# UoB-HPC/stdpar-nbody

Hardware: AMD Instinct MI355X
Metric: body-steps/sec + %FP64 peak, 3D double all-pairs N=2^20 at 1/2/4/8 GPUs (higher is better)
Workload: dtype f64

## Files before the change

stdpar-nbody_amd/csrc/all_pairs.hip:

```cpp
#include "common.hpp"
#include "k1_order_key.hpp"
#include "radix_sort.hpp"

#include <atomic>
#include <cstdlib>
#include <mutex>
#include <type_traits>
#include <vector>

namespace nbody {

constexpr int kBlock = 256;
constexpr int kWaves = kBlock / 64;

struct ap_config {
  int split = 0;
  int tpt   = 0;
  int path  = 0;
};
static std::atomic<uint32_t> g_ap_default{0};

static ap_config ap_config_of(const nbody_state* s) {
  const uint32_t t = s->tuning ? s->tuning : g_ap_default.load(std::memory_order_relaxed);
  ap_config c;
// ... 24 lines not shown

template <typename T, int D>
__global__ __launch_bounds__(kBlock) void pack_sources_kernel(const T* __restrict__ m, const T* __restrict__ x,
                                                              src_rec<T, D>* __restrict__ out, uint32_t sz, uint32_t padded) {
  const uint32_t j = blockIdx.x * kBlock + threadIdx.x;
  if (j >= padded) return;
  src_rec<T, D> r;
#pragma unroll
  for (int k = 0; k < 3; ++k) r.p[k] = (k < D && j < sz) ? x[uint64_t(j) * D + (k < D ? k : 0)] : T(0);
  r.m    = j < sz ? m[j] : T(0);
  out[j] = r;
}

template <typename T>
struct k1_prepare_tail {
  uint32_t turn_words;
};
template <>
struct k1_prepare_tail<double> {
  uint32_t turn_words;
  uint32_t bpc;
  double* cbox;
  double* pbox;
};
template <typename T, int D, bool PACK, bool MOMENTS>
__global__ __launch_bounds__(kBlock) void k1_prepare_kernel(const T* __restrict__ m, const T* __restrict__ x, src_rec<T, D>* __restrict__ out,
                                                            cst_batch* __restrict__ cst, uint32_t sz, uint32_t padded, k1_rule* rule, double* partial,
                                                            uint32_t* turn, k1_prepare_tail<T> tail) {
  constexpr bool BOX        = PACK && MOMENTS && sizeof(T) == 8;
  const uint32_t turn_words = tail.turn_words;
  [[maybe_unused]] uint32_t bpc = 0;
  [[maybe_unused]] T *cbox = nullptr, *pbox = nullptr;
  if constexpr (BOX) bpc = tail.bpc, cbox = tail.cbox, pbox = tail.pbox;
  const uint32_t j = blockIdx.x * kBlock + threadIdx.x;
  T p[D];
#pragma unroll
  for (int k = 0; k < D; ++k) p[k] = j < sz ? x[uint64_t(j) * D + k] : T(0);
  if constexpr (PACK) {
    if (j < padded) {
      src_rec<T, D> r;
#pragma unroll
      for (int k = 0; k < 3; ++k) r.p[k] = k < D ? p[k < D ? k : 0] : T(0);
      r.m    = j < sz ? m[j] : T(0);
      out[j] = r;
      if constexpr (sizeof(T) == 8) {
        const src_cst<T> k  = src_cst<T>::of(r.m);
        cst[j / 2].m15[j % 2]   = k.m15;
        cst[j / 2].m1875[j % 2] = k.m1875;
      }
    }
  }
  __shared__ double red[2 * D][kWaves];
  __shared__ T bred[BOX ? 2 * D : 1][kWaves];
  __shared__ bool last_s;
  const int lane = threadIdx.x & 63, wave = threadIdx.x >> 6;
  if constexpr (MOMENTS) {
// ... 84 lines not shown
    __syncthreads();
    if (threadIdx.x < 2 * D) {
      double tot = 0.0;
#pragma unroll 6
      for (int gg = 0; gg < G; ++gg) tot += fin[gg * (2 * D) + threadIdx.x];
      fin[threadIdx.x] = tot;
    }
    __syncthreads();
    if (threadIdx.x == 0) {
      double vol = 1.0;
#pragma unroll
      for (int k = 0; k < D; ++k) {
        const double mean = fin[k] / double(sz), var = fin[D + k] / double(sz) - mean * mean;
        vol *= var > 0.0 ? __builtin_sqrt(12.0 * var) : 0.0;
      }
      rule->volume = vol;
      rule->sparse = vol >= kFarMinVolume<D> ? 1u : 0u;
    }
  }
  if constexpr (BOX) {
    if (bpc != 0) {
      const uint32_t nchunks = (gridDim.x + bpc - 1) / bpc;
      const uint32_t sub     = threadIdx.x & 15u;
      for (uint32_t c0 = 0; c0 < nchunks; c0 += kBlock / 16) {
        const uint32_t c  = c0 + (threadIdx.x >> 4);
        const uint32_t b1 = c < nchunks ? min(gridDim.x, (c + 1u) * bpc) : 0u;
        T lo[D], hi[D];
#pragma unroll
        for (int k = 0; k < D; ++k) lo[k] = T(__builtin_inf()), hi[k] = -T(__builtin_inf());
        for (uint32_t b0 = c * bpc + sub; b0 < b1; b0 += 16u * 4u) {
          T v[4][2 * D];
#pragma unroll
          for (int u = 0; u < 4; ++u) {
            const uint32_t b = b0 + 16u * uint32_t(u);
#pragma unroll
            for (int q = 0; q < 2 * D; ++q)
              v[u][q] = b < b1 ? __hip_atomic_load(pbox + size_t(b) * (2 * D) + q, __ATOMIC_RELAXED, __HIP_MEMORY_SCOPE_AGENT)
                               : (q < D ? T(__builtin_inf()) : -T(__builtin_inf()));
          }
#pragma unroll
          for (int u = 0; u < 4; ++u)
#pragma unroll
            for (int k = 0; k < D; ++k) {
              lo[k] = __builtin_fmin(lo[k], v[u][k]);
              hi[k] = __builtin_fmax(hi[k], v[u][D + k]);
            }
        }
#pragma unroll
        for (int k = 0; k < D; ++k)
          for (int off = 8; off > 0; off >>= 1) {
            lo[k] = __builtin_fmin(lo[k], __shfl_xor(lo[k], off, 64));
            hi[k] = __builtin_fmax(hi[k], __shfl_xor(hi[k], off, 64));
          }
        if (c < nchunks && sub == 0) {
#pragma unroll
          for (int k = 0; k < D; ++k) {
            cbox[size_t(c) * (2 * D) + k]     = lo[k];
            cbox[size_t(c) * (2 * D) + D + k] = hi[k];
          }
        }
      }
    }
  }
  for (uint32_t w = threadIdx.x; w < turn_words; w += kBlock) turn[w] = 0u;
  if (threadIdx.x == 0) __hip_atomic_store(&rule->ticket, 0u, __ATOMIC_RELAXED, __HIP_MEMORY_SCOPE_AGENT);
}

template <int JS>
constexpr int kSgprWaves = JS > kWaves ? JS : kWaves;

constexpr uint32_t kTurnSpins  = 1u << 26;
constexpr uint32_t kTurnPoison = 0xffffffffu;
struct k1_status {
  uint32_t err, block, group, chunk;
  unsigned long long polls, waits;
};
struct k1_handoff {
  void* sums;
  uint32_t* turn;
  k1_status* status;
  uint32_t spins;
  uint32_t delay;
  uint32_t late;
};
constexpr size_t kBoxHeaderBytes = 64;
template <typename T>
struct k1_rule_arg {
  const k1_rule* rule;
};
template <>
struct k1_rule_arg<double> {
  const k1_rule* rule;
  const double* box;
};
template <typename T, int D, int R, int JS, int RULE = 0>
__global__ __launch_bounds__(64 * kSgprWaves<JS>) void all_pairs_force_sgpr_kernel(const src_rec<T, D>* __restrict__ packed,
                                                                                   const cst_batch* __restrict__ cst,
                                                                                   const T* __restrict__ x, T* a, T c, uint32_t sz,
                                                                                   uint32_t first, uint32_t count,
                                                                                   uint32_t tiles_per_chunk, k1_handoff h,
                                                                                   k1_rule_arg<T> ra) {
  [[maybe_unused]] constexpr T e2 = T(0);
  const k1_rule* __restrict__ const rule = ra.rule;
  [[maybe_unused]] const T* __restrict__ box = nullptr;
  if constexpr (sizeof(T) == 8) box = ra.box;
#define K1_SOFT false
#include "k1_sgpr_body.inc"
#undef K1_SOFT
}
template <typename T, int D, int R, int JS>
__global__ __launch_bounds__(64 * kSgprWaves<JS>) void all_pairs_softened_sgpr_kernel(const src_rec<T, D>* __restrict__ packed,
                                                                                      const cst_batch* __restrict__ cst,
                                                                                      const T* __restrict__ x, T* a, T c, uint32_t sz,
                                                                                      uint32_t first, uint32_t count,
                                                                                      uint32_t tiles_per_chunk, k1_handoff h, T e2) {
  constexpr int RULE = 0;
  const k1_rule* const rule = nullptr;
  [[maybe_unused]] const T* const box = nullptr;
#define K1_SOFT true
#include "k1_sgpr_body.inc"
#undef K1_SOFT
}

namespace {
struct scratch_buf {
  void* ptr  = nullptr;
  size_t cap = 0;
};
struct packed_slot {
  int device;
  hipStream_t stream;
  scratch_buf buf[9];
  std::vector<void*> retired;
  bool k1_dirty  = false;
  bool k1_failed = false;
};
std::mutex g_packed_mu;
std::vector<packed_slot> g_packed_slots;
}

int ap_scratch_get(hipStream_t st, int which, size_t bytes, void** out) {
// ... 101 lines not shown
  void* scratch         = nullptr;
  if (int r = ap_scratch_get(st, 0, 4 * tsz * size_t(padded), &scratch)) return r;
  int rc = dispatch(s->dtype, s->dim, [&](auto tg) {
    using T         = typename decltype(tg)::type;
    constexpr int D = decltype(tg)::dim;
    hipLaunchKernelGGL((pack_sources_kernel<T, D>), dim3((padded + kBlock - 1) / kBlock), dim3(kBlock), 0, st,
                       static_cast<const T*>(s->m), static_cast<const T*>(s->x), static_cast<src_rec<T, D>*>(scratch), s->sz, padded);
    NB_HIP(hipGetLastError());
    return int(NBODY_OK);
  });
  *packed_out = scratch;
  return rc;
}

static size_t ap_cst_bytes(size_t padded) { return sizeof(cst_batch) * (padded / 2); }

static size_t ap_rule_bytes(uint32_t sz, int dim) {
  const size_t padded = (size_t(sz) + kTileJ - 1) / kTileJ * kTileJ;
  return 32 + sizeof(double) * 2 * size_t(dim) * (padded / kBlock);
}

static size_t ap_box_bytes(uint32_t sz, int dim) {
  const size_t ntiles = (size_t(sz) + kTileJ - 1) / kTileJ;
  return kBoxHeaderBytes + sizeof(double) * 2 * size_t(dim) * (ntiles + ntiles * (kTileJ / kBlock));
}
static bool k1_box_wanted(uint32_t sz, uint32_t chunks) { return sz >= kFarMinBodies && chunks > 1; }

constexpr double kOrderSafe = 1e150;
__device__ __forceinline__ double k1_order_safe(double p, bool on) { return on && p > kOrderSafe ? kOrderSafe : (on && p < -kOrderSafe ? -kOrderSafe : p); }
constexpr uint32_t kOrderMinBodies = 262144;
static bool k1_order_wanted(uint32_t sz, uint32_t chunks) {
  if (const char* e = experiment_env("NBODY_K1_NO_ORDER"); e && e[0] == '1') return false;
  uint32_t least = kOrderMinBodies;
  if (const char* e = experiment_env("NBODY_K1_ORDER_MIN")) least = uint32_t(strtoul(e, nullptr, 10));
  return k1_box_wanted(sz, chunks) && sz >= least;
}

struct k1_order_layout {
  size_t recs, cst, keys[2], idx[2], hist, xs, as, bytes;
};
static k1_order_layout k1_order_layout_of(uint32_t sz, uint32_t count, int dim) {
  const size_t padded = (size_t(sz) + kTileJ - 1) / kTileJ * kTileJ;
  size_t at           = 0;
  auto take = [&](size_t bytes) {
    const size_t here = at;
    at += (bytes + 255) / 256 * 256;
    return here;
// ... 54 lines not shown
    for (int off = 32; off > 0; off >>= 1) {
      lo[k] = __builtin_fmin(lo[k], __shfl_xor(lo[k], off, 64));
      hi[k] = __builtin_fmax(hi[k], __shfl_xor(hi[k], off, 64));
    }
  __shared__ double bred[2 * D][kWaves];
  const int lane = threadIdx.x & 63, wave = threadIdx.x >> 6;
  if (lane == 0) {
#pragma unroll
    for (int k = 0; k < D; ++k) {
      bred[k][wave]     = lo[k];
      bred[D + k][wave] = hi[k];
    }
  }
  __syncthreads();
  if (threadIdx.x < 2 * D) {
    const int q = int(threadIdx.x);
    double v    = bred[q][0];
    for (int w = 1; w < kWaves; ++w) v = q < D ? __builtin_fmin(v, bred[q][w]) : __builtin_fmax(v, bred[q][w]);
    pbox[size_t(blockIdx.x) * (2 * D) + q] = v;
  }
}

template <int D>
__global__ __launch_bounds__(kBlock) void k1_order_box_kernel(const double* __restrict__ pbox, uint32_t nblk, uint32_t bpc, double* __restrict__ cbox) {
  const uint32_t b0 = blockIdx.x * bpc, b1 = min(nblk, b0 + bpc);
  double lo[D], hi[D];
#pragma unroll
  for (int k = 0; k < D; ++k) lo[k] = __builtin_inf(), hi[k] = -__builtin_inf();
  for (uint32_t b = b0 + threadIdx.x; b < b1; b += kBlock) {
#pragma unroll
    for (int k = 0; k < D; ++k) {
      lo[k] = __builtin_fmin(lo[k], pbox[size_t(b) * (2 * D) + k]);
      hi[k] = __builtin_fmax(hi[k], pbox[size_t(b) * (2 * D) + D + k]);
    }
  }
#pragma unroll
  for (int k = 0; k < D; ++k)
    for (int off = 32; off > 0; off >>= 1) {
      lo[k] = __builtin_fmin(lo[k], __shfl_xor(lo[k], off, 64));
      hi[k] = __builtin_fmax(hi[k], __shfl_xor(hi[k], off, 64));
    }
  __shared__ double bred[2 * D][kWaves];
  const int lane = threadIdx.x & 63, wave = threadIdx.x >> 6;
  if (lane == 0) {
#pragma unroll
    for (int k = 0; k < D; ++k) {
      bred[k][wave]     = lo[k];
      bred[D + k][wave] = hi[k];
    }
  }
  __syncthreads();
  if (threadIdx.x < 2 * D) {
    const int q = int(threadIdx.x);
    double v    = bred[q][0];
    for (int w = 1; w < kWaves; ++w) v = q < D ? __builtin_fmin(v, bred[q][w]) : __builtin_fmax(v, bred[q][w]);
    cbox[size_t(blockIdx.x) * (2 * D) + q] = v;
  }
}

template <int D>
__global__ __launch_bounds__(kBlock) void k1_order_targets_kernel(const double* __restrict__ x, uint32_t first, uint32_t count,
                                                                  const uint32_t* __restrict__ perm, double* __restrict__ xs,
                                                                  const k1_rule* __restrict__ rule) {
  const uint32_t k = blockIdx.x * kBlock + threadIdx.x;
  if (k >= count) return;
  const uint64_t i = uint64_t(first) + perm[k];
  const bool safe  = rule->sparse != 0u;
#pragma unroll
  for (int d = 0; d < D; ++d) xs[uint64_t(k) * D + d] = k1_order_safe(x[i * D + d], safe);
}

template <int D>
__global__ __launch_bounds__(kBlock) void k1_order_scatter_kernel(const uint64_t* __restrict__ as, uint32_t count, const uint32_t* __restrict__ perm,
                                                                  uint64_t* __restrict__ a) {
  const uint32_t k = blockIdx.x * kBlock + threadIdx.x;
  if (k >= count) return;
  const uint64_t i = perm[k];
#pragma unroll
  for (int d = 0; d < D; ++d) a[i * D + d] = as[uint64_t(k) * D + d];
}

template <int D>
struct k1_ordered {
  src_rec<double, D>* packed;
  const cst_batch* cst;
  const double* box;
  const double* xs;
  double* as;
  const uint32_t* tperm;
};

template <int D>
static int k1_order_queue(const nbody_state* s, hipStream_t st, const src_rec<double, D>* packed, const cst_batch* cst, const k1_rule* rule,
                          uint32_t tpc, k1_ordered<D>* out) {
  const uint32_t padded = (s->sz + kTileJ - 1) / kTileJ * kTileJ, nblk = padded / kBlock, bpc = tpc * (kTileJ / kBlock);
  const k1_order_layout l = k1_order_layout_of(s->sz, s->count, D);
  void *w = nullptr, *b = nullptr;
  if (int r = ap_scratch_get(st, 8, l.bytes, &w)) return r;
  if (int r = ap_scratch_get(st, 7, ap_box_bytes(s->sz, D), &b)) return r;
  char* base = static_cast<char*>(w);
  uint64_t* keys[2] = {reinterpret_cast<uint64_t*>(base + l.keys[0]), reinterpret_cast<uint64_t*>(base + l.keys[1])};
  uint32_t* idx[2]  = {reinterpret_cast<uint32_t*>(base + l.idx[0]), reinterpret_cast<uint32_t*>(base + l.idx[1])};
  uint32_t* hist    = reinterpret_cast<uint32_t*>(base + l.hist);
  auto* recs        = reinterpret_cast<src_rec<double, D>*>(base + l.recs);
  auto* csts        = reinterpret_cast<cst_batch*>(base + l.cst);
  double* xs        = reinterpret_cast<double*>(base + l.xs);
  double* cbox      = reinterpret_cast<double*>(static_cast<char*>(b) + kBoxHeaderBytes);
  double* pbox      = cbox + size_t(2 * D) * (padded / kTileJ);
  const double* x   = static_cast<const double*>(s->x);
  const bool whole  = s->first == 0 && s->count == s->sz;
  int fin           = 0;
  hipLaunchKernelGGL((k1_order_key_kernel<D>), dim3((s->sz + kBlock - 1) / kBlock), dim3(kBlock), 0, st, x, 0u, s->sz, rule, keys[0]);
  NB_HIP(hipGetLastError());
  if (int r = radix_sort_pairs(keys, idx, s->sz, kOrderKeyBits, hist, st, &fin)) return r;
  hipLaunchKernelGGL((k1_order_gather_kernel<D>), dim3(nblk), dim3(kBlock), 0, st, packed, cst, idx[fin], recs, csts, s->sz, pbox,
                     whole ? xs : static_cast<double*>(nullptr), rule);
  NB_HIP(hipGetLastError());
  hipLaunchKernelGGL((k1_order_box_kernel<D>), dim3((nblk + bpc - 1) / bpc), dim3(kBlock), 0, st, pbox, nblk, bpc, cbox);
  NB_HIP(hipGetLastError());
  if (!whole) {
    hipLaunchKernelGGL((k1_order_key_kernel<D>), dim3((s->count + kBlock - 1) / kBlock), dim3(kBlock), 0, st, x, s->first, s->count, rule, keys[0]);
    NB_HIP(hipGetLastError());
    if (int r = radix_sort_pairs(keys, idx, s->count, kOrderKeyBits, hist, st, &fin)) return r;
    hipLaunchKernelGGL((k1_order_targets_kernel<D>), dim3((s->count + kBlock - 1) / kBlock), dim3(kBlock), 0, st, x, s->first, s->count, idx[fin], xs, rule);
    NB_HIP(hipGetLastError());
  }
  *out = {recs, csts, cbox, xs, reinterpret_cast<double*>(base + l.as), idx[fin]};
  return NBODY_OK;
}

template <typename T, int D>
static int ap_prepare(const nbody_state* s, hipStream_t st, bool pack, src_rec<T, D>** packed_out, const cst_batch** cst_out,
                      const k1_rule** rule_out, uint32_t* turn, size_t turn_words, bool with_rule = true, uint32_t box_tpc = 0,
                      const T** box_out = nullptr) {
  const uint32_t padded = (s->sz + kTileJ - 1) / kTileJ * kTileJ;
  const bool moments    = with_rule && s->sz >= kFarMinBodies;
  void* scratch         = nullptr;
  void* consts          = nullptr;
  if (pack) {
    if (int r = ap_scratch_get(st, 0, 4 * sizeof(T) * size_t(padded), &scratch)) return r;
    if (sizeof(T) == 8)
      if (int r = ap_scratch_get(st, 6, ap_cst_bytes(padded), &consts)) return r;
  }
  void* q = nullptr;
  if (int r = ap_scratch_get(st, 3, ap_rule_bytes(s->sz, D), &q)) return r;
  auto* rule    = static_cast<k1_rule*>(q);
  auto* partial = reinterpret_cast<double*>(static_cast<char*>(q) + 32);
  auto* out     = static_cast<src_rec<T, D>*>(scratch);
  auto* cst     = static_cast<cst_batch*>(consts);
  T *cbox = nullptr, *pbox = nullptr;
  uint32_t bpc = 0;
  if (sizeof(T) == 8 && pack && moments && box_tpc != 0) {
    void* b = nullptr;
    if (int r = ap_scratch_get(st, 7, ap_box_bytes(s->sz, D), &b)) return r;
    cbox = reinterpret_cast<T*>(static_cast<char*>(b) + kBoxHeaderBytes);
    pbox = cbox + size_t(2 * D) * (padded / kTileJ);
    bpc  = box_tpc * (kTileJ / kBlock);
  }
  const dim3 grid(padded / kBlock), block(kBlock);
  const T *m = static_cast<const T*>(s->m), *x = static_cast<const T*>(s->x);
  const uint32_t words = uint32_t(turn_words);
  k1_prepare_tail<T> tail{};
  tail.turn_words = words;
  if constexpr (sizeof(T) == 8) tail.bpc = bpc, tail.cbox = cbox, tail.pbox = pbox;
  if (pack && moments) hipLaunchKernelGGL((k1_prepare_kernel<T, D, true, true>), grid, block, 0, st, m, x, out, cst, s->sz, padded, rule, partial, turn, tail);
  else if (pack) hipLaunchKernelGGL((k1_prepare_kernel<T, D, true, false>), grid, block, 0, st, m, x, out, cst, s->sz, padded, rule, partial, turn, tail);
  else if (moments) hipLaunchKernelGGL((k1_prepare_kernel<T, D, false, true>), grid, block, 0, st, m, x, out, cst, s->sz, padded, rule, partial, turn, tail);
  NB_HIP(hipGetLastError());
  if (box_out) *box_out = cbox;
  if (packed_out) *packed_out = out;
  if (cst_out) *cst_out = cst;
  *rule_out = moments ? rule : nullptr;
  return NBODY_OK;
}

constexpr uint32_t kCollectMaxBlocks = 2048;
static bool k1_collect(uint32_t target_blocks, uint32_t chunks) {
  uint32_t limit = kCollectMaxBlocks;
  if (const char* e = experiment_env("NBODY_K1_COLLECT_MAX")) limit = uint32_t(atoi(e));
  return chunks > 1 && uint64_t(target_blocks) * chunks <= limit;
}
template <typename T, int D, int R, int JS>
static size_t k1_collect_bytes(uint32_t target_blocks, uint32_t chunks) {
  constexpr int TG = kSgprWaves<JS> / JS;
  return sizeof(T) * size_t(chunks) * target_blocks * TG * R * D * 64;
}

template <int R, int JS>
static size_t sgpr_turn_words(uint32_t count) {
  constexpr int TG = kSgprWaves<JS> / JS, TB = TG * 64 * R;
  return size_t((count + TB - 1) / TB) * TG;
}
// ... 7 lines not shown
  if (plan.chunks > 1) {
    void* q = nullptr;
    if (int r = ap_scratch_get(st, 1, sizeof(uint32_t) * sgpr_turn_words<R, JS>(s->count), &q)) return r;
    h.turn = static_cast<uint32_t*>(q);
    if (k1_collect(blocks, plan.chunks)) {
      if (int r = ap_scratch_get(st, 5, k1_collect_bytes<T, D, R, JS>(blocks, plan.chunks), &q)) return r;
      h.sums = q;
    }
    if (int r = ap_scratch_get(st, 4, sizeof(k1_status), &q)) return r;
    h.status = static_cast<k1_status*>(q);
    if (const char* e = experiment_env("NBODY_K1_TURN_SPINS")) h.spins = uint32_t(strtoul(e, nullptr, 10));
    if (const char* e = experiment_env("NBODY_K1_HANDOFF_DELAY")) h.delay = uint32_t(strtoul(e, nullptr, 10));
    if (const char* e = experiment_env("NBODY_K1_HANDOFF_LATE")) h.late = uint32_t(strtoul(e, nullptr, 10));
    if (const char* e = experiment_env("NBODY_K1_NO_HANDOFF"); e && e[0] == '1') h.turn = nullptr, h.sums = nullptr;
    if (const char* e = experiment_env("NBODY_K1_COLLECT"); e && e[0] == '0') h.sums = nullptr;
  }
  src_rec<T, D>* packed = nullptr;
  const cst_batch* cst  = nullptr;
  const k1_rule* rule   = nullptr;
  const T* box          = nullptr;
  bool certify          = !SOFT && sizeof(T) == 8 && k1_box_wanted(s->sz, plan.chunks);
  if (const char* e = experiment_env("NBODY_K1_NO_CERT"); e && e[0] == '1') certify = false;
  [[maybe_unused]] const bool ordered = certify && plan.chunks > 1 && k1_order_wanted(s->sz, plan.chunks);
  if (int r = ap_prepare<T, D>(s, st, true, &packed, &cst, &rule, h.turn, h.turn ? sgpr_turn_words<R, JS>(s->count) : 0, !SOFT,
                               certify && !ordered ? plan.tiles_per_chunk : 0u, &box))
    return r;
  if constexpr (SOFT) {
    hipLaunchKernelGGL((all_pairs_softened_sgpr_kernel<T, D, R, JS>), dim3(blocks, plan.chunks), dim3(64 * kSgprWaves<JS>), 0, st,
                       packed, cst, static_cast<const T*>(s->x), static_cast<T*>(s->a), static_cast<T>(s->c), s->sz, s->first, s->count,
                       plan.tiles_per_chunk, h, e2);
    NB_HIP(hipGetLastError());
    if (h.turn != nullptr && h.sums == nullptr) ap_status_mark(st);
    return NBODY_OK;
  }
  k1_rule_arg<T> ra{};
  ra.rule = rule;
  if constexpr (sizeof(T) == 8) ra.box = box;
#ifdef NBODY_EXPERIMENTS
  if (const char* e = getenv("NBODY_K1_RULE_FORCE"); e && JS == 8 && D == 3) {
    if (e[0] == '1')
      hipLaunchKernelGGL((all_pairs_force_sgpr_kernel<T, D, R, JS, 1>), dim3(blocks, plan.chunks), dim3(64 * kSgprWaves<JS>), 0, st,
                         packed, cst, static_cast<const T*>(s->x), static_cast<T*>(s->a), static_cast<T>(s->c), s->sz, s->first, s->count,
                         plan.tiles_per_chunk, h, ra);
    else
      hipLaunchKernelGGL((all_pairs_force_sgpr_kernel<T, D, R, JS, 2>), dim3(blocks, plan.chunks), dim3(64 * kSgprWaves<JS>), 0, st,
                         packed, cst, static_cast<const T*>(s->x), static_cast<T*>(s->a), static_cast<T>(s->c), s->sz, s->first, s->count,
                         plan.tiles_per_chunk, h, ra);
    NB_HIP(hipGetLastError());
    return NBODY_OK;
  }
#endif
  if constexpr (sizeof(T) == 8) {
    if (ordered) {
      k1_ordered<D> o{};
      if (int r = k1_order_queue<D>(s, st, packed, cst, rule, plan.tiles_per_chunk, &o)) return r;
      ra.box = o.box;
      hipLaunchKernelGGL((all_pairs_force_sgpr_kernel<T, D, R, JS>), dim3(blocks, plan.chunks), dim3(64 * kSgprWaves<JS>), 0, st,
                         o.packed, o.cst, o.xs, o.as, static_cast<T>(s->c), s->sz, 0u, s->count, plan.tiles_per_chunk, h, ra);
      NB_HIP(hipGetLastError());
      hipLaunchKernelGGL((k1_order_scatter_kernel<D>), dim3((s->count + kBlock - 1) / kBlock), dim3(kBlock), 0, st,
                         reinterpret_cast<const uint64_t*>(o.as), s->count, o.tperm, static_cast<uint64_t*>(s->a));
      NB_HIP(hipGetLastError());
      if (h.turn != nullptr && h.sums == nullptr) ap_status_mark(st);
      return NBODY_OK;
    }
  }
  hipLaunchKernelGGL((all_pairs_force_sgpr_kernel<T, D, R, JS>), dim3(blocks, plan.chunks), dim3(64 * kSgprWaves<JS>), 0, st,
                     packed, cst, static_cast<const T*>(s->x), static_cast<T*>(s->a), static_cast<T>(s->c), s->sz, s->first, s->count,
                     plan.tiles_per_chunk, h, ra);
  NB_HIP(hipGetLastError());
  if (h.turn != nullptr && h.sums == nullptr) ap_status_mark(st);
  return NBODY_OK;
}

template <typename T, int D, int R, int JS, bool SOFT>
static int launch_all_pairs(const nbody_state* s, hipStream_t st, T e2) {
  constexpr int TB = (kWaves / JS) * 64 * R;
  uint32_t blocks  = (s->count + TB - 1) / TB;
  if (blocks == 0) return NBODY_OK;
// ... 42 lines not shown
    rc = p.scalar ? launch_all_pairs_sgpr<T, D, R, JS, SOFT>(s, p, st, e2)
                  : (JS <= kWaves ? launch_all_pairs<T, D, R, (JS <= kWaves ? JS : 1), SOFT>(s, st, e2) : int(NBODY_ERR_ARG));
  });
  if (!found) {
    set_error("all-pairs: unsupported config split=%d targets_per_thread=%d", p.js, p.r);
    return NBODY_ERR_ARG;
  }
  return rc;
}

template <typename T, int D>
static int all_pairs_describe(const nbody_state* s, char* out, size_t len) {
  k1_plan p;
  if (int rc = plan_all_pairs<T>(s, &p)) return rc;
  const char* t = sizeof(T) == 8 ? "double" : "float";
  const char* pair = sizeof(T) == 4 ? (s->sz >= kFarMinBodies ? "rsq+rcp[m y^3 at r2 >= 4 if sparse]" : "rsq+rcp")
                                    : s->sz >= kFarMinBodies ? "far3m[-eps if sparse]/near3" : "far3m/near3";
  if (p.scalar) {
    bool collect = false;
    with_k1_instance(p, [&](auto r, auto js) {
      constexpr int TB = (kSgprWaves<decltype(js)::value> / decltype(js)::value) * 64 * decltype(r)::value;
      collect = k1_collect((s->count + TB - 1) / TB, p.chunks);
    });
    snprintf(out, len, "all_pairs_force_sgpr_kernel<%s,%d,R=%d,JS=%d> tile=%d chunks=%u%s pair=%s%s", t, D, p.r, p.js, kTileJ, p.chunks,
             p.chunks > 1 ? (collect ? "(summed in chunk order by the last to arrive)" : "(summed in turn into a)") : "", pair,
             sizeof(T) == 8 && k1_box_wanted(s->sz, p.chunks)
                 ? (k1_order_wanted(s->sz, p.chunks) ? " cert=box-gap>=3[if sparse: blocks proven far skip the r2 test] order=morton30[if sparse]"
                                                    : " cert=box-gap>=3[if sparse: blocks proven far skip the r2 test]")
                 : "");
  }
  else
    snprintf(out, len, "all_pairs_force_kernel<%s,%d,R=%d,JS=%d> tile=%d chunks=1 pair=%s", t, D, p.r, p.js, kTileJ, pair);
  return NBODY_OK;
}

int ap_scratch_reserve(hipStream_t st, const nbody_state* s) {
  void* q             = nullptr;
  const size_t tsz    = s->dtype == NBODY_F32 ? 4 : 8;
  const size_t padded = (size_t(s->sz) + 2 * kTileJ - 1) / (2 * kTileJ) * (2 * kTileJ);
  if (int r = ap_scratch_get(st, 0, 4 * tsz * padded, &q)) return r;
  if (s->dtype == NBODY_F64)
    if (int r = ap_scratch_get(st, 6, ap_cst_bytes(padded), &q)) return r;
  if (int r = ap_scratch_get(st, 3, ap_rule_bytes(s->sz, s->dim), &q)) return r;
  if (s->dtype == NBODY_F64 && s->sz >= kFarMinBodies)
    if (int r = ap_scratch_get(st, 7, ap_box_bytes(s->sz, s->dim), &q)) return r;
  if (s->dtype == NBODY_F64) {
    k1_plan p;
    if (int rc = plan_all_pairs<double>(s, &p)) return rc;
    if (p.scalar && k1_order_wanted(s->sz, p.chunks))
      if (int r = ap_scratch_get(st, 8, k1_order_layout_of(s->sz, s->count, s->dim).bytes, &q)) return r;
  }
  return dispatch(s->dtype, s->dim, [&](auto tg) {
// ... 653 lines not shown

extern "C" int nbody_all_pairs_softened_force(const nbody_state* s, double eps, void* stream) {
  if (int r = check_state(s)) return r;
  return dispatch(s->dtype, s->dim, [&](auto tg) {
    using TG = decltype(tg);
    using T  = typename TG::type;
    T e2;
    if (int r = check_softening<T>(eps, &e2)) return r;
    device_guard guard(stream_device(as_stream(stream)));
    return all_pairs_dispatch<T, TG::dim, true>(s, as_stream(stream), e2);
  });
}

extern "C" int nbody_all_pairs_status(void* stream, uint64_t out[6], int clear) {
  device_guard guard(stream_device(as_stream(stream)));
  unsigned long long v[6] = {0, 0, 0, 0, 0, 0};
  const int rc = ap_status_read(as_stream(stream), v, clear != 0);
  if (out)
    for (int i = 0; i < 6; ++i) out[i] = v[i];
  return rc;
}

#ifdef NBODY_EXPERIMENTS
extern "C" int nbody_exp_k1_certified(void* stream, uint64_t* out, int clear) {
  NB_ARG(out != nullptr, "out is NULL");
  hipStream_t st = as_stream(stream);
  const int dev  = stream_device(st);
  device_guard guard(dev);
  void* dptr = nullptr;
  {
    std::lock_guard<std::mutex> lock(g_packed_mu);
    for (auto& sl : g_packed_slots)
      if (sl.stream == st && sl.device == dev) dptr = sl.buf[7].ptr;
  }
  unsigned long long v = 0;
  if (dptr) NB_HIP(hipMemcpyAsync(&v, dptr, sizeof v, hipMemcpyDeviceToHost, st));
  NB_HIP(hipStreamSynchronize(st));
  if (dptr && clear) {
    NB_HIP(hipMemsetAsync(dptr, 0, sizeof v, st));
    NB_HIP(hipStreamSynchronize(st));
  }
  *out = v;
  return NBODY_OK;
}
#endif

extern "C" int nbody_all_pairs_collapsed_force(const nbody_state* s, void* stream) {
  if (int r = check_state(s)) return r;
  device_guard guard(stream_device(as_stream(stream)));
  return dispatch(s->dtype, s->dim, [&](auto tg) {
    using TG = decltype(tg);
    return collapsed_dispatch<typename TG::type, TG::dim>(s, as_stream(stream));
  });
}

extern "C" int nbody_accelerate_step(const nbody_state* s, void* stream) {
  if (int r = check_state(s)) return r;
// ... 7 lines not shown
```

stdpar-nbody_amd/csrc/k1_sgpr_body.inc:

```
  using rec_t = src_rec<T, D>;
  constexpr int TG  = kSgprWaves<JS> / JS;
  constexpr int TB  = TG * 64 * R;
  constexpr int SUB = kTileJ / JS;
  __shared__ T partial[(JS > 1) ? (JS - 1) * TG * 64 * R * D : 1];
  const int lane   = threadIdx.x & 63;
  const int wave   = __builtin_amdgcn_readfirstlane(threadIdx.x >> 6);
  const int tgroup = wave / JS;
  const int jpart  = wave % JS;
  T xi[R][D], acc[R][D];
  uint32_t ti[R];
#pragma unroll
  for (int r = 0; r < R; ++r) {
    uint32_t local = blockIdx.x * TB + tgroup * (64 * R) + r * 64 + lane;
    ti[r]          = local;
    uint64_t i     = uint64_t(first) + (local < count ? local : 0u);
#pragma unroll
    for (int k = 0; k < D; ++k) {
      xi[r][k]  = x[i * D + k];
      acc[r][k] = T(0);
    }
  }
  const uint32_t ntiles = (sz + kTileJ - 1) / kTileJ;
  const uint32_t t0     = blockIdx.y * tiles_per_chunk;
  const uint32_t t1     = min(ntiles, t0 + tiles_per_chunk);
  const pair_consts<T> pc;
  const bool ffar       = !K1_SOFT && ap_far_mode(rule);
  const uint32_t nsteps = (t1 - t0) * SUB;
  constexpr int U = 64 / int(sizeof(rec_t));
  struct batch_t {
    rec_t r[U];
  };
  auto batch = [&](uint32_t k) { return packed + (uint64_t(t0 + k / SUB) * kTileJ + uint32_t(jpart) * SUB + (k % SUB)); };
  constexpr bool CST = sizeof(T) == 8;
  auto cbatch = [&](uint32_t k) { return cst + (uint64_t(t0 + k / SUB) * kTileJ + uint32_t(jpart) * SUB + (k % SUB)) / U; };
  [[maybe_unused]] uint32_t vzero = 0;
  if constexpr (CST) {
    asm volatile("" : "+v"(vzero));
#pragma unroll
    for (int r = 0; r < R; ++r)
#pragma unroll
      for (int k = 0; k < D; ++k) asm volatile("" : "+v"(xi[r][k]));
  }
  [[maybe_unused]] bool cfar = false;
  if constexpr (!K1_SOFT && CST && RULE == 0) {
    if (ffar && box != nullptr) {
      cfar = k1_block_is_far<T, D, R>(xi, (const T __attribute__((address_space(4)))*)(box + size_t(blockIdx.y) * (2 * D)));
#ifdef NBODY_EXPERIMENTS
      if (cfar && jpart == 0 && lane == 0)
        atomicAdd(reinterpret_cast<unsigned long long*>(const_cast<T*>(box)) - kBoxHeaderBytes / 8, 1ull);
#endif
    }
  }
  auto run = [&](auto ff) {
    constexpr int FF = int(decltype(ff)::value);
    sgpr16 A, B;
    [[maybe_unused]] cst_regs CA, CB;
    auto request = [&](sgpr16& S, cst_regs& C, uint32_t k) {
      if constexpr (CST) C = cload(cbatch(k), vzero, xi[0][0]);
      S = sload16(batch(k), xi[0][0]);
    };
    auto wait = [&](sgpr16& S, cst_regs& C) {
      if constexpr (CST) cswait(S, C, acc[0][0]);
      else swait(S, acc[0][0]);
    };
    auto consume = [&](const sgpr16& S, const cst_regs& C) {
      const batch_t b = __builtin_bit_cast(batch_t, S);
      src_cst<T> kc[U];
      if constexpr (CST) cst_unpack(C, kc);
      if constexpr (K1_SOFT) pair_batch_soft<T, D, R, U, true>(acc, xi, b.r, kc, pc, e2);
      else if constexpr (FF == 2) pair_batch_far<T, D, R, U>(acc, xi, b.r, kc);
      else pair_batch<T, D, R, U, FF != 0>(acc, xi, b.r, kc, pc);
    };
    request(A, CA, 0);
    for (uint32_t k = 0; k < nsteps; k += 2 * U) {
      wait(A, CA);
      request(B, CB, k + U);
      consume(A, CA);
      wait(B, CB);
      request(A, CA, k + 2 * U < nsteps ? k + 2 * U : k);
      consume(B, CB);
    }
    wait(A, CA);
  };
  if constexpr (K1_SOFT) run(std::false_type{});
  else if constexpr (RULE == 1) run(std::false_type{});
  else if constexpr (RULE == 2) run(std::true_type{});
  else if (ffar) {
    if constexpr (CST) {
      if (cfar) run(std::integral_constant<int, 2>{});
      else run(std::true_type{});
    } else run(std::true_type{});
  } else run(std::false_type{});
  if constexpr (JS > 1) {
    if (jpart > 0) {
#pragma unroll
      for (int r = 0; r < R; ++r)
#pragma unroll
        for (int k = 0; k < D; ++k) partial[((((jpart - 1) * TG + tgroup) * R + r) * D + k) * 64 + lane] = acc[r][k];
    }
    __syncthreads();
    if (jpart == 0) {
#pragma unroll
      for (int p = 1; p < JS; ++p)
#pragma unroll
        for (int r = 0; r < R; ++r)
#pragma unroll
          for (int k = 0; k < D; ++k) acc[r][k] += partial[((((p - 1) * TG + tgroup) * R + r) * D + k) * 64 + lane];
    }
  }
  if (jpart != 0) return;
  const uint32_t y = blockIdx.y, last = gridDim.y - 1u;
  uint32_t* const tw = h.turn + blockIdx.x * TG + tgroup;
  if (h.sums != nullptr) {
    const size_t group_scalars = size_t(R) * D * 64;
    T* const all  = static_cast<T*>(h.sums);
// ... 112 lines not shown
```

Before: 1.829 million.

## Certify far-field at finer tile-run granularity to skip distance tests per run

Adds per-run bounding boxes (groups of tiles within a chunk) computed in the prepare and order-box kernels. When a whole chunk is not proven far, the force kernel now tests each run separately and uses the cheaper far-field pair routine for runs proven far, splitting the main loop into segments. This aims to skip more r2 tests in sparse configurations, at the cost of extra box reduction work, more box checks per block, and a segmented loop with a restarted prefetch pipeline at each run boundary.

```diff
diff --git a/stdpar-nbody_amd/csrc/all_pairs.hip b/stdpar-nbody_amd/csrc/all_pairs.hip
--- a/stdpar-nbody_amd/csrc/all_pairs.hip
+++ b/stdpar-nbody_amd/csrc/all_pairs.hip
@@ -70,6 +70,9 @@
   uint32_t bpc;
   double* cbox;
   double* pbox;
+  uint32_t bpr;
+  uint32_t rpc;
+  double* rbox;
 };
 template <typename T, int D, bool PACK, bool MOMENTS>
 __global__ __launch_bounds__(kBlock) void k1_prepare_kernel(const T* __restrict__ m, const T* __restrict__ x, src_rec<T, D>* __restrict__ out,
@@ -78,8 +81,9 @@
   constexpr bool BOX        = PACK && MOMENTS && sizeof(T) == 8;
   const uint32_t turn_words = tail.turn_words;
   [[maybe_unused]] uint32_t bpc = 0;
-  [[maybe_unused]] T *cbox = nullptr, *pbox = nullptr;
-  if constexpr (BOX) bpc = tail.bpc, cbox = tail.cbox, pbox = tail.pbox;
+  [[maybe_unused]] T *cbox = nullptr, *pbox = nullptr, *rbox = nullptr;
+  [[maybe_unused]] uint32_t bpr = 0, rpc = 1;
+  if constexpr (BOX) bpc = tail.bpc, cbox = tail.cbox, pbox = tail.pbox, bpr = tail.bpr, rpc = tail.rpc, rbox = tail.rbox;
   const uint32_t j = blockIdx.x * kBlock + threadIdx.x;
   T p[D];
 #pragma unroll
@@ -210,44 +214,50 @@
     if (bpc != 0) {
       const uint32_t nchunks = (gridDim.x + bpc - 1) / bpc;
       const uint32_t sub     = threadIdx.x & 15u;
-      for (uint32_t c0 = 0; c0 < nchunks; c0 += kBlock / 16) {
-        const uint32_t c  = c0 + (threadIdx.x >> 4);
-        const uint32_t b1 = c < nchunks ? min(gridDim.x, (c + 1u) * bpc) : 0u;
-        T lo[D], hi[D];
-#pragma unroll
-        for (int k = 0; k < D; ++k) lo[k] = T(__builtin_inf()), hi[k] = -T(__builtin_inf());
-        for (uint32_t b0 = c * bpc + sub; b0 < b1; b0 += 16u * 4u) {
-          T v[4][2 * D];
-#pragma unroll
-          for (int u = 0; u < 4; ++u) {
-            const uint32_t b = b0 + 16u * uint32_t(u);
-#pragma unroll
-            for (int q = 0; q < 2 * D; ++q)
-              v[u][q] = b < b1 ? __hip_atomic_load(pbox + size_t(b) * (2 * D) + q, __ATOMIC_RELAXED, __HIP_MEMORY_SCOPE_AGENT)
-                               : (q < D ? T(__builtin_inf()) : -T(__builtin_inf()));
+      auto reduce = [&](uint32_t per, uint32_t width, T* dst) {
+        const uint32_t units = nchunks * per;
+        for (uint32_t c0 = 0; c0 < units; c0 += kBlock / 16) {
+          const uint32_t c  = c0 + (threadIdx.x >> 4);
+          const uint32_t at = (c / per) * bpc + (c % per) * width;
+          const uint32_t b1 = c < units ? min(gridDim.x, min(at + width, (c / per + 1u) * bpc)) : 0u;
+          T lo[D], hi[D];
+#pragma unroll
+          for (int k = 0; k < D; ++k) lo[k] = T(__builtin_inf()), hi[k] = -T(__builtin_inf());
+          for (uint32_t b0 = at + sub; b0 < b1; b0 += 16u * 4u) {
+            T v[4][2 * D];
+#pragma unroll
+            for (int u = 0; u < 4; ++u) {
+              const uint32_t b = b0 + 16u * uint32_t(u);
+#pragma unroll
+              for (int q = 0; q < 2 * D; ++q)
+                v[u][q] = b < b1 ? __hip_atomic_load(pbox + size_t(b) * (2 * D) + q, __ATOMIC_RELAXED, __HIP_MEMORY_SCOPE_AGENT)
+                                 : (q < D ? T(__builtin_inf()) : -T(__builtin_inf()));
+            }
+#pragma unroll
+            for (int u = 0; u < 4; ++u)
+#pragma unroll
+              for (int k = 0; k < D; ++k) {
+                lo[k] = __builtin_fmin(lo[k], v[u][k]);
+                hi[k] = __builtin_fmax(hi[k], v[u][D + k]);
+              }
           }
 #pragma unroll
-          for (int u = 0; u < 4; ++u)
+          for (int k = 0; k < D; ++k)
+            for (int off = 8; off > 0; off >>= 1) {
+              lo[k] = __builtin_fmin(lo[k], __shfl_xor(lo[k], off, 64));
+              hi[k] = __builtin_fmax(hi[k], __shfl_xor(hi[k], off, 64));
+            }
+          if (c < units && sub == 0) {
 #pragma unroll
             for (int k = 0; k < D; ++k) {
-              lo[k] = __builtin_fmin(lo[k], v[u][k]);
-              hi[k] = __builtin_fmax(hi[k], v[u][D + k]);
+              dst[size_t(c) * (2 * D) + k]     = lo[k];
+              dst[size_t(c) * (2 * D) + D + k] = hi[k];
             }
-        }
-#pragma unroll
-        for (int k = 0; k < D; ++k)
-          for (int off = 8; off > 0; off >>= 1) {
-            lo[k] = __builtin_fmin(lo[k], __shfl_xor(lo[k], off, 64));
-            hi[k] = __builtin_fmax(hi[k], __shfl_xor(hi[k], off, 64));
-          }
-        if (c < nchunks && sub == 0) {
-#pragma unroll
-          for (int k = 0; k < D; ++k) {
-            cbox[size_t(c) * (2 * D) + k]     = lo[k];
-            cbox[size_t(c) * (2 * D) + D + k] = hi[k];
           }
         }
-      }
+      };
+      reduce(1u, bpc, cbox);
+      if (bpr != 0) reduce(rpc, bpr, rbox);
     }
   }
   for (uint32_t w = threadIdx.x; w < turn_words; w += kBlock) turn[w] = 0u;
@@ -280,7 +290,25 @@
 struct k1_rule_arg<double> {
   const k1_rule* rule;
   const double* box;
+  const double* rbox;
+  uint32_t cert_tiles;
+  uint32_t runs_per_chunk;
 };
+constexpr uint32_t kCertTiles = 16;
+struct k1_runs {
+  uint32_t tiles = 0, per_chunk = 1;
+};
+static k1_runs k1_runs_of(uint32_t tiles_per_chunk) {
+  uint32_t ct = kCertTiles;
+  if (const char* e = experiment_env("NBODY_K1_CERT_TILES")) ct = uint32_t(atoi(e));
+  const uint32_t least = (tiles_per_chunk + 63) / 64;
+  if (ct < least) ct = least;
+  k1_runs r;
+  if (ct == 0 || ct >= tiles_per_chunk) return r;
+  r.tiles     = ct;
+  r.per_chunk = (tiles_per_chunk + ct - 1) / ct;
+  return r;
+}
 template <typename T, int D, int R, int JS, int RULE = 0>
 __global__ __launch_bounds__(64 * kSgprWaves<JS>) void all_pairs_force_sgpr_kernel(const src_rec<T, D>* __restrict__ packed,
                                                                                    const cst_batch* __restrict__ cst,
@@ -291,7 +319,9 @@
   [[maybe_unused]] constexpr T e2 = T(0);
   const k1_rule* __restrict__ const rule = ra.rule;
   [[maybe_unused]] const T* __restrict__ box = nullptr;
-  if constexpr (sizeof(T) == 8) box = ra.box;
+  [[maybe_unused]] const T* __restrict__ rbox = nullptr;
+  [[maybe_unused]] uint32_t cert_tiles = 0, runs_per_chunk = 1;
+  if constexpr (sizeof(T) == 8) box = ra.box, rbox = ra.rbox, cert_tiles = ra.cert_tiles, runs_per_chunk = ra.runs_per_chunk;
 #define K1_SOFT false
 #include "k1_sgpr_body.inc"
 #undef K1_SOFT
@@ -304,7 +334,8 @@
                                                                                       uint32_t tiles_per_chunk, k1_handoff h, T e2) {
   constexpr int RULE = 0;
   const k1_rule* const rule = nullptr;
-  [[maybe_unused]] const T* const box = nullptr;
+  [[maybe_unused]] const T *const box = nullptr, *const rbox = nullptr;
+  [[maybe_unused]] constexpr uint32_t cert_tiles = 1, runs_per_chunk = 1;
 #define K1_SOFT true
 #include "k1_sgpr_body.inc"
 #undef K1_SOFT
@@ -452,7 +483,14 @@
 
 static size_t ap_box_bytes(uint32_t sz, int dim) {
   const size_t ntiles = (size_t(sz) + kTileJ - 1) / kTileJ;
-  return kBoxHeaderBytes + sizeof(double) * 2 * size_t(dim) * (ntiles + ntiles * (kTileJ / kBlock));
+  return kBoxHeaderBytes + sizeof(double) * 2 * size_t(dim) * (ntiles + ntiles * (kTileJ / kBlock) + 2 * ntiles + 2);
+}
+template <int D>
+static void ap_box_arrays(void* buf, uint32_t sz, double** cbox, double** pbox, double** rbox) {
+  const size_t ntiles = (size_t(sz) + kTileJ - 1) / kTileJ;
+  *cbox = reinterpret_cast<double*>(static_cast<char*>(buf) + kBoxHeaderBytes);
+  *pbox = *cbox + size_t(2 * D) * ntiles;
+  *rbox = *pbox + size_t(2 * D) * ntiles * (kTileJ / kBlock);
 }
 static bool k1_box_wanted(uint32_t sz, uint32_t chunks) { return sz >= kFarMinBodies && chunks > 1; }
 
@@ -553,8 +591,13 @@
 }
 
 template <int D>
-__global__ __launch_bounds__(kBlock) void k1_order_box_kernel(const double* __restrict__ pbox, uint32_t nblk, uint32_t bpc, double* __restrict__ cbox) {
-  const uint32_t b0 = blockIdx.x * bpc, b1 = min(nblk, b0 + bpc);
+__global__ __launch_bounds__(kBlock) void k1_order_box_kernel(const double* __restrict__ pbox, uint32_t nblk, uint32_t bpc, double* __restrict__ cbox,
+                                                              uint32_t nchunks, uint32_t bpr, uint32_t rpc, double* __restrict__ rbox) {
+  const bool is_run = blockIdx.x >= nchunks;
+  const uint32_t u  = is_run ? blockIdx.x - nchunks : blockIdx.x;
+  const uint32_t c  = is_run ? u / rpc : u;
+  const uint32_t b0 = c * bpc + (is_run ? (u % rpc) * bpr : 0u), b1 = min(nblk, min(b0 + (is_run ? bpr : bpc), (c + 1u) * bpc));
+  double* const dst = is_run ? rbox : cbox;
   double lo[D], hi[D];
 #pragma unroll
   for (int k = 0; k < D; ++k) lo[k] = __builtin_inf(), hi[k] = -__builtin_inf();
@@ -585,7 +628,7 @@
     const int q = int(threadIdx.x);
     double v    = bred[q][0];
     for (int w = 1; w < kWaves; ++w) v = q < D ? __builtin_fmin(v, bred[q][w]) : __builtin_fmax(v, bred[q][w]);
-    cbox[size_t(blockIdx.x) * (2 * D) + q] = v;
+    dst[size_t(u) * (2 * D) + q] = v;
   }
 }
 
@@ -616,6 +659,7 @@
   src_rec<double, D>* packed;
   const cst_batch* cst;
   const double* box;
+  const double* rbox;
   const double* xs;
   double* as;
   const uint32_t* tperm;
@@ -623,7 +667,7 @@
 
 template <int D>
 static int k1_order_queue(const nbody_state* s, hipStream_t st, const src_rec<double, D>* packed, const cst_batch* cst, const k1_rule* rule,
-                          uint32_t tpc, k1_ordered<D>* out) {
+                          uint32_t tpc, const k1_runs& runs, k1_ordered<D>* out) {
   const uint32_t padded = (s->sz + kTileJ - 1) / kTileJ * kTileJ, nblk = padded / kBlock, bpc = tpc * (kTileJ / kBlock);
   const k1_order_layout l = k1_order_layout_of(s->sz, s->count, D);
   void *w = nullptr, *b = nullptr;
@@ -636,8 +680,9 @@
   auto* recs        = reinterpret_cast<src_rec<double, D>*>(base + l.recs);
   auto* csts        = reinterpret_cast<cst_batch*>(base + l.cst);
   double* xs        = reinterpret_cast<double*>(base + l.xs);
-  double* cbox      = reinterpret_cast<double*>(static_cast<char*>(b) + kBoxHeaderBytes);
-  double* pbox      = cbox + size_t(2 * D) * (padded / kTileJ);
+  double *cbox = nullptr, *pbox = nullptr, *rbox = nullptr;
+  ap_box_arrays<D>(b, s->sz, &cbox, &pbox, &rbox);
+  const uint32_t nchunks = (nblk + bpc - 1) / bpc, bpr = runs.tiles * (kTileJ / kBlock);
   const double* x   = static_cast<const double*>(s->x);
   const bool whole  = s->first == 0 && s->count == s->sz;
   int fin           = 0;
@@ -647,7 +692,8 @@
   hipLaunchKernelGGL((k1_order_gather_kernel<D>), dim3(nblk), dim3(kBlock), 0, st, packed, cst, idx[fin], recs, csts, s->sz, pbox,
                      whole ? xs : static_cast<double*>(nullptr), rule);
   NB_HIP(hipGetLastError());
-  hipLaunchKernelGGL((k1_order_box_kernel<D>), dim3((nblk + bpc - 1) / bpc), dim3(kBlock), 0, st, pbox, nblk, bpc, cbox);
+  hipLaunchKernelGGL((k1_order_box_kernel<D>), dim3(nchunks + (bpr ? nchunks * runs.per_chunk : 0u)), dim3(kBlock), 0, st, pbox, nblk, bpc, cbox,
+                     nchunks, bpr, runs.per_chunk, rbox);
   NB_HIP(hipGetLastError());
   if (!whole) {
     hipLaunchKernelGGL((k1_order_key_kernel<D>), dim3((s->count + kBlock - 1) / kBlock), dim3(kBlock), 0, st, x, s->first, s->count, rule, keys[0]);
@@ -656,14 +702,14 @@
     hipLaunchKernelGGL((k1_order_targets_kernel<D>), dim3((s->count + kBlock - 1) / kBlock), dim3(kBlock), 0, st, x, s->first, s->count, idx[fin], xs, rule);
     NB_HIP(hipGetLastError());
   }
-  *out = {recs, csts, cbox, xs, reinterpret_cast<double*>(base + l.as), idx[fin]};
+  *out = {recs, csts, cbox, bpr ? rbox : nullptr, xs, reinterpret_cast<double*>(base + l.as), idx[fin]};
   return NBODY_OK;
 }
 
 template <typename T, int D>
 static int ap_prepare(const nbody_state* s, hipStream_t st, bool pack, src_rec<T, D>** packed_out, const cst_batch** cst_out,
                       const k1_rule** rule_out, uint32_t* turn, size_t turn_words, bool with_rule = true, uint32_t box_tpc = 0,
-                      const T** box_out = nullptr) {
+                      const T** box_out = nullptr, const k1_runs& runs = k1_runs(), const T** rbox_out = nullptr) {
   const uint32_t padded = (s->sz + kTileJ - 1) / kTileJ * kTileJ;
   const bool moments    = with_rule && s->sz >= kFarMinBodies;
   void* scratch         = nullptr;
@@ -679,26 +725,31 @@
   auto* partial = reinterpret_cast<double*>(static_cast<char*>(q) + 32);
   auto* out     = static_cast<src_rec<T, D>*>(scratch);
   auto* cst     = static_cast<cst_batch*>(consts);
-  T *cbox = nullptr, *pbox = nullptr;
-  uint32_t bpc = 0;
-  if (sizeof(T) == 8 && pack && moments && box_tpc != 0) {
-    void* b = nullptr;
-    if (int r = ap_scratch_get(st, 7, ap_box_bytes(s->sz, D), &b)) return r;
-    cbox = reinterpret_cast<T*>(static_cast<char*>(b) + kBoxHeaderBytes);
-    pbox = cbox + size_t(2 * D) * (padded / kTileJ);
-    bpc  = box_tpc * (kTileJ / kBlock);
+  [[maybe_unused]] double *cbox = nullptr, *pbox = nullptr, *rbox = nullptr;
+  uint32_t bpc = 0, bpr = 0;
+  if constexpr (sizeof(T) == 8) {
+    if (pack && moments && box_tpc != 0) {
+      void* b = nullptr;
+      if (int r = ap_scratch_get(st, 7, ap_box_bytes(s->sz, D), &b)) return r;
+      ap_box_arrays<D>(b, s->sz, &cbox, &pbox, &rbox);
+      bpc = box_tpc * (kTileJ / kBlock);
+      bpr = runs.tiles * (kTileJ / kBlock);
+    }
   }
   const dim3 grid(padded / kBlock), block(kBlock);
   const T *m = static_cast<const T*>(s->m), *x = static_cast<const T*>(s->x);
   const uint32_t words = uint32_t(turn_words);
   k1_prepare_tail<T> tail{};
   tail.turn_words = words;
-  if constexpr (sizeof(T) == 8) tail.bpc = bpc, tail.cbox = cbox, tail.pbox = pbox;
+  if constexpr (sizeof(T) == 8) tail.bpc = bpc, tail.cbox = cbox, tail.pbox = pbox, tail.bpr = bpr, tail.rpc = runs.per_chunk, tail.rbox = rbox;
   if (pack && moments) hipLaunchKernelGGL((k1_prepare_kernel<T, D, true, true>), grid, block, 0, st, m, x, out, cst, s->sz, padded, rule, partial, turn, tail);
   else if (pack) hipLaunchKernelGGL((k1_prepare_kernel<T, D, true, false>), grid, block, 0, st, m, x, out, cst, s->sz, padded, rule, partial, turn, tail);
   else if (moments) hipLaunchKernelGGL((k1_prepare_kernel<T, D, false, true>), grid, block, 0, st, m, x, out, cst, s->sz, padded, rule, partial, turn, tail);
   NB_HIP(hipGetLastError());
-  if (box_out) *box_out = cbox;
+  if constexpr (sizeof(T) == 8) {
+    if (box_out) *box_out = cbox;
+    if (rbox_out) *rbox_out = bpr ? rbox : nullptr;
+  }
   if (packed_out) *packed_out = out;
   if (cst_out) *cst_out = cst;
   *rule_out = moments ? rule : nullptr;
@@ -752,8 +803,10 @@
   bool certify          = !SOFT && sizeof(T) == 8 && k1_box_wanted(s->sz, plan.chunks);
   if (const char* e = experiment_env("NBODY_K1_NO_CERT"); e && e[0] == '1') certify = false;
   [[maybe_unused]] const bool ordered = certify && plan.chunks > 1 && k1_order_wanted(s->sz, plan.chunks);
+  const k1_runs runs = certify ? k1_runs_of(plan.tiles_per_chunk) : k1_runs();
+  const T* rbox      = nullptr;
   if (int r = ap_prepare<T, D>(s, st, true, &packed, &cst, &rule, h.turn, h.turn ? sgpr_turn_words<R, JS>(s->count) : 0, !SOFT,
-                               certify && !ordered ? plan.tiles_per_chunk : 0u, &box))
+                               certify && !ordered ? plan.tiles_per_chunk : 0u, &box, runs, &rbox))
     return r;
   if constexpr (SOFT) {
     hipLaunchKernelGGL((all_pairs_softened_sgpr_kernel<T, D, R, JS>), dim3(blocks, plan.chunks), dim3(64 * kSgprWaves<JS>), 0, st,
@@ -765,7 +818,7 @@
   }
   k1_rule_arg<T> ra{};
   ra.rule = rule;
-  if constexpr (sizeof(T) == 8) ra.box = box;
+  if constexpr (sizeof(T) == 8) ra.box = box, ra.rbox = rbox, ra.cert_tiles = runs.tiles, ra.runs_per_chunk = runs.per_chunk;
 #ifdef NBODY_EXPERIMENTS
   if (const char* e = getenv("NBODY_K1_RULE_FORCE"); e && JS == 8 && D == 3) {
     if (e[0] == '1')
@@ -783,8 +836,8 @@
   if constexpr (sizeof(T) == 8) {
     if (ordered) {
       k1_ordered<D> o{};
-      if (int r = k1_order_queue<D>(s, st, packed, cst, rule, plan.tiles_per_chunk, &o)) return r;
-      ra.box = o.box;
+      if (int r = k1_order_queue<D>(s, st, packed, cst, rule, plan.tiles_per_chunk, runs, &o)) return r;
+      ra.box = o.box, ra.rbox = o.rbox;
       hipLaunchKernelGGL((all_pairs_force_sgpr_kernel<T, D, R, JS>), dim3(blocks, plan.chunks), dim3(64 * kSgprWaves<JS>), 0, st,
                          o.packed, o.cst, o.xs, o.as, static_cast<T>(s->c), s->sz, 0u, s->count, plan.tiles_per_chunk, h, ra);
       NB_HIP(hipGetLastError());
@@ -873,12 +926,15 @@
       constexpr int TB = (kSgprWaves<decltype(js)::value> / decltype(js)::value) * 64 * decltype(r)::value;
       collect = k1_collect((s->count + TB - 1) / TB, p.chunks);
     });
-    snprintf(out, len, "all_pairs_force_sgpr_kernel<%s,%d,R=%d,JS=%d> tile=%d chunks=%u%s pair=%s%s", t, D, p.r, p.js, kTileJ, p.chunks,
-             p.chunks > 1 ? (collect ? "(summed in chunk order by the last to arrive)" : "(summed in turn into a)") : "", pair,
-             sizeof(T) == 8 && k1_box_wanted(s->sz, p.chunks)
-                 ? (k1_order_wanted(s->sz, p.chunks) ? " cert=box-gap>=3[if sparse: blocks proven far skip the r2 test] order=morton30[if sparse]"
-                                                    : " cert=box-gap>=3[if sparse: blocks proven far skip the r2 test]")
-                 : "");
+    const bool boxes = sizeof(T) == 8 && k1_box_wanted(s->sz, p.chunks);
+    const k1_runs runs = boxes ? k1_runs_of(p.tiles_per_chunk) : k1_runs();
+    char cert[160]     = "";
+    if (boxes && runs.tiles)
+      snprintf(cert, sizeof cert, " cert=box-gap>=3 per %u tiles[if sparse: blocks, else their runs of tiles, proven far skip the r2 test]", runs.tiles);
+    else if (boxes) snprintf(cert, sizeof cert, " cert=box-gap>=3[if sparse: blocks proven far skip the r2 test]");
+    snprintf(out, len, "all_pairs_force_sgpr_kernel<%s,%d,R=%d,JS=%d> tile=%d chunks=%u%s pair=%s%s%s", t, D, p.r, p.js, kTileJ, p.chunks,
+             p.chunks > 1 ? (collect ? "(summed in chunk order by the last to arrive)" : "(summed in turn into a)") : "", pair, cert,
+             boxes && k1_order_wanted(s->sz, p.chunks) ? " order=morton30[if sparse]" : "");
   }
   else
     snprintf(out, len, "all_pairs_force_kernel<%s,%d,R=%d,JS=%d> tile=%d chunks=1 pair=%s", t, D, p.r, p.js, kTileJ, pair);
@@ -1578,7 +1634,10 @@
 }
 
 #ifdef NBODY_EXPERIMENTS
-extern "C" int nbody_exp_k1_certified(void* stream, uint64_t* out, int clear) {
+static int k1_certified_word(void* stream, int word, uint64_t* out, int clear);
+extern "C" int nbody_exp_k1_certified(void* stream, uint64_t* out, int clear) { return k1_certified_word(stream, 0, out, clear); }
+extern "C" int nbody_exp_k1_certified_runs(void* stream, uint64_t* out, int clear) { return k1_certified_word(stream, 1, out, clear); }
+static int k1_certified_word(void* stream, int word, uint64_t* out, int clear) {
   NB_ARG(out != nullptr, "out is NULL");
   hipStream_t st = as_stream(stream);
   const int dev  = stream_device(st);
@@ -1589,6 +1648,7 @@
     for (auto& sl : g_packed_slots)
       if (sl.stream == st && sl.device == dev) dptr = sl.buf[7].ptr;
   }
+  if (dptr) dptr = static_cast<unsigned long long*>(dptr) + word;
   unsigned long long v = 0;
   if (dptr) NB_HIP(hipMemcpyAsync(&v, dptr, sizeof v, hipMemcpyDeviceToHost, st));
   NB_HIP(hipStreamSynchronize(st));
diff --git a/stdpar-nbody_amd/csrc/k1_sgpr_body.inc b/stdpar-nbody_amd/csrc/k1_sgpr_body.inc
--- a/stdpar-nbody_amd/csrc/k1_sgpr_body.inc
+++ b/stdpar-nbody_amd/csrc/k1_sgpr_body.inc
@@ -41,17 +41,31 @@
 #pragma unroll
       for (int k = 0; k < D; ++k) asm volatile("" : "+v"(xi[r][k]));
   }
-  [[maybe_unused]] bool cfar = false;
+  [[maybe_unused]] bool cfar       = false;
+  [[maybe_unused]] uint64_t rfar   = 0;
+  [[maybe_unused]] uint32_t rsteps = nsteps;
   if constexpr (!K1_SOFT && CST && RULE == 0) {
     if (ffar && box != nullptr) {
       cfar = k1_block_is_far<T, D, R>(xi, (const T __attribute__((address_space(4)))*)(box + size_t(blockIdx.y) * (2 * D)));
+      if (!cfar && rbox != nullptr) {
+        const T* rb = rbox + size_t(blockIdx.y) * runs_per_chunk * (2 * D);
+        uint32_t r  = 0;
+        for (uint32_t t = t0; t < t1; t += cert_tiles, ++r, rb += 2 * D)
+          rfar |= uint64_t(k1_block_is_far<T, D, R>(xi, (const T __attribute__((address_space(4)))*)rb)) << r;
+        rsteps = cert_tiles * SUB;
+      }
 #ifdef NBODY_EXPERIMENTS
-      if (cfar && jpart == 0 && lane == 0)
-        atomicAdd(reinterpret_cast<unsigned long long*>(const_cast<T*>(box)) - kBoxHeaderBytes / 8, 1ull);
+      if (jpart == 0 && lane == 0) {
+        unsigned long long* const counts = reinterpret_cast<unsigned long long*>(const_cast<T*>(box)) - kBoxHeaderBytes / 8;
+        if (cfar) atomicAdd(counts, 1ull);
+        const uint32_t nruns = rbox != nullptr ? (t1 - t0 + cert_tiles - 1) / cert_tiles : 1u;
+        const uint32_t got   = cfar ? nruns : uint32_t(__builtin_popcountll(rfar));
+        if (got) atomicAdd(counts + 1, (unsigned long long)got);
+      }
 #endif
     }
   }
-  auto run = [&](auto ff) {
+  auto run = [&](auto ff, uint32_t k0, uint32_t k1) {
     constexpr int FF = int(decltype(ff)::value);
     sgpr16 A, B;
     [[maybe_unused]] cst_regs CA, CB;
@@ -71,26 +85,36 @@
       else if constexpr (FF == 2) pair_batch_far<T, D, R, U>(acc, xi, b.r, kc);
       else pair_batch<T, D, R, U, FF != 0>(acc, xi, b.r, kc, pc);
     };
-    request(A, CA, 0);
-    for (uint32_t k = 0; k < nsteps; k += 2 * U) {
+    request(A, CA, k0);
+    for (uint32_t k = k0; k < k1; k += 2 * U) {
       wait(A, CA);
       request(B, CB, k + U);
       consume(A, CA);
       wait(B, CB);
-      request(A, CA, k + 2 * U < nsteps ? k + 2 * U : k);
+      request(A, CA, k + 2 * U < k1 ? k + 2 * U : k);
       consume(B, CB);
     }
     wait(A, CA);
   };
-  if constexpr (K1_SOFT) run(std::false_type{});
-  else if constexpr (RULE == 1) run(std::false_type{});
-  else if constexpr (RULE == 2) run(std::true_type{});
+  if constexpr (K1_SOFT) run(std::false_type{}, 0u, nsteps);
+  else if constexpr (RULE == 1) run(std::false_type{}, 0u, nsteps);
+  else if constexpr (RULE == 2) run(std::true_type{}, 0u, nsteps);
   else if (ffar) {
     if constexpr (CST) {
-      if (cfar) run(std::integral_constant<int, 2>{});
-      else run(std::true_type{});
-    } else run(std::true_type{});
-  } else run(std::false_type{});
+      const uint64_t bits = cfar ? ~0ull : rfar;
+      uint32_t r = 0, k0 = 0;
+      do {
+        const uint64_t far  = (bits >> r) & 1ull;
+        const uint64_t rest = (bits ^ (0ull - far)) >> r;
+        r += rest ? uint32_t(__builtin_ctzll(rest)) : 64u;
+        const uint32_t end = r * rsteps;
+        const uint32_t k1  = r < 64u && end < nsteps ? end : nsteps;
+        if (far) run(std::integral_constant<int, 2>{}, k0, k1);
+        else run(std::true_type{}, k0, k1);
+        k0 = k1;
+      } while (k0 < nsteps);
+    } else run(std::true_type{}, 0u, nsteps);
+  } else run(std::false_type{}, 0u, nsteps);
   if constexpr (JS > 1) {
     if (jpart > 0) {
 #pragma unroll
```

New measurement: 1.841 million, median of 6. About the same (+0.6%).
